# AsherBond/0-kno-vectorx

Measured on AMD Instinct MI355X. Metric: header_range_256 proofs/sec, higher is better.
Workload: dtype u64 (Goldilocks) / u8 (hashes)

## Files before the change

### 0-kno-vectorx_amd/csrc/vx_blake_air.hip

```cpp
#include <string.h>

#include "air_blake.cuh"
#include "vx_internal.h"


static uint8_t compact_mode(uint32_t v) { return v < (1u << 6) ? 0 : v < (1u << 14) ? 1 : v < (1u << 30) ? 2 : 3; }

struct BlockDesc {
    uint64_t msg_off;
    uint32_t t, inc;
    uint32_t D[8];
    uint8_t fin, first, act, mode;
    uint32_t num;
    uint32_t size;
};

__device__ __forceinline__ uint64_t b_rotr(uint64_t x, int n) { return (x >> n) | (x << (64 - n)); }

__device__ __forceinline__ void carries(uint64_t o1, uint64_t o2, uint64_t o3, uint8_t* out) {
    uint64_t lo = (o1 & 0xFFFFFFFFULL) + (o2 & 0xFFFFFFFFULL) + (o3 & 0xFFFFFFFFULL);
    uint64_t klo = lo >> 32;
    uint64_t hi = (o1 >> 32) + (o2 >> 32) + (o3 >> 32) + klo;
    out[0] = (uint8_t)klo;
    out[1] = (uint8_t)(hi >> 32);
}
__device__ __forceinline__ void g_mix(uint64_t* v, int ia, int ib, int ic, int id, uint64_t x, uint64_t y) {
    uint64_t a = v[ia], b = v[ib], c = v[ic], d = v[id];
    uint64_t a1 = a + b + x, d1 = b_rotr(d ^ a1, 32), c1 = c + d1, b1 = b_rotr(b ^ c1, 24);
    uint64_t a2 = a1 + b1 + y, d2 = b_rotr(d1 ^ a2, 16), c2 = c1 + d2, b2 = b_rotr(b1 ^ c2, 63);
    v[ia] = a2, v[ib] = b2, v[ic] = c2, v[id] = d2;
}
__device__ void blake_round(uint64_t* v, const uint64_t* m, int round) {
    const uint8_t* s = blk::ORDER[round + 1];
    for (int k = 0; k < 4; ++k) g_mix(v, k, 4 + k, 8 + k, 12 + k, m[s[2 * k]], m[s[2 * k + 1]]);
    for (int j = 0; j < 4; ++j) g_mix(v, j, 4 + (j + 1) % 4, 8 + (j + 2) % 4, 12 + (j + 3) % 4, m[s[8 + 2 * j]], m[s[8 + 2 * j + 1]]);
}
__device__ void blake_init_v(uint64_t* v, const uint64_t* h, uint64_t t, bool fin) {
    for (int i = 0; i < 8; ++i) v[i] = h[i], v[8 + i] = blk::IV[i];
    v[12] ^= t;
    if (fin) v[14] = ~v[14];
}

__global__ __launch_bounds__(64) void k_blake_chain(const uint8_t* msgs, size_t stride, const uint32_t* sizes, size_t n,
                                                    const uint32_t* block_base, uint64_t* hchain, uint8_t* digests) {
    size_t i = blockIdx.x * (size_t)blockDim.x + threadIdx.x;
    if (i >= n) return;
    const uint64_t* p = (const uint64_t*)(msgs + i * stride);
    const uint32_t len = sizes[i];
    const uint32_t nchunks = len == 0 ? 1 : (len + 127) / 128;
    uint64_t h[8], m[16], v[16];
    for (int k = 0; k < 8; ++k) h[k] = blk::IV[k];
    h[0] ^= 0x01010020ULL;
    for (uint32_t cidx = 0; cidx < nchunks; ++cidx) {
        uint64_t* hc = hchain + 8 * ((size_t)block_base[i] + cidx);
        for (int k = 0; k < 8; ++k) hc[k] = h[k];
        const bool fin = cidx + 1 == nchunks;
        const uint32_t off = 128 * cidx, rem = fin ? len - off : 128;
        for (int k = 0; k < 16; ++k) {
            uint32_t b = 8 * k;
            uint64_t w = 0;
            if (b < rem) {
                w = p[(off >> 3) + k];
                if (rem - b < 8) w &= (1ULL << (8 * (rem - b))) - 1;
            }
            m[k] = w;
        }
        blake_init_v(v, h, fin ? len : off + 128, fin);
        for (int r = 0; r < 12; ++r) blake_round(v, m, r);
        for (int k = 0; k < 8; ++k) h[k] ^= v[k] ^ v[k + 8];
    }
    uint64_t* d = (uint64_t*)(digests + 32 * i);
    d[0] = h[0], d[1] = h[1], d[2] = h[2], d[3] = h[3];
}

#ifndef VX_HIST_COPIES
#define VX_HIST_COPIES 8
#endif
constexpr int HIST_COPIES = VX_HIST_COPIES;
constexpr int SW_CAR = 64, SW_MS = 65, SW_MB = 81, SW_HL = 82, SW_D = 90, SW_FLAGS = 94, SW_TN = 95, SW_WIN = 96, N_STAGE = 97;
struct ExpandEntry {
    uint16_t col;
    uint8_t shift, bits;
};
__global__ __launch_bounds__(256) void k_blake_trace(const uint8_t* msgs, const BlockDesc* descs, const uint64_t* hchain, size_t n_real,
                                                     uint64_t* __restrict__ stage, uint32_t* __restrict__ hist, uint32_t* __restrict__ rc_part, size_t n,
                                                     uint32_t win_off, uint32_t win_len) {
    using namespace blk;
    __shared__ uint32_t rc_lds[256];
    rc_lds[threadIdx.x] = 0;
    __syncthreads();
    const size_t row = blockIdx.x * (size_t)blockDim.x + threadIdx.x;
    const size_t b = row >> 4;
    const int r = (int)(row & 15);
    const BlockDesc d = descs[b];
    uint64_t h[8], m[16], v[16];
    if (b < n_real) {
        for (int k = 0; k < 8; ++k) h[k] = hchain[8 * b + k];
        const uint64_t* p = (const uint64_t*)(msgs + d.msg_off);
        for (int k = 0; k < 16; ++k) {
            uint32_t bb = 8 * k;
            uint64_t w = 0;
            if (bb < d.inc) {
                w = p[k];
                if (d.inc - bb < 8) w &= (1ULL << (8 * (d.inc - bb))) - 1;
            }
            m[k] = w;
        }
    } else {
        for (int k = 0; k < 8; ++k) h[k] = IV[k];
        h[0] ^= 0x01010020ULL;
        for (int k = 0; k < 16; ++k) m[k] = k < 4 ? ((uint64_t)d.D[2 * k] | ((uint64_t)d.D[2 * k + 1] << 32)) : 0;
        m[4] = d.mode == 0 ? 4ULL * d.num : d.mode == 1 ? 4ULL * d.num + 1 : d.mode == 2 ? 4ULL * d.num + 2 : (3ULL | ((uint64_t)d.num << 8));
    }
    auto st = [&](int w) -> uint64_t& { return stage[(size_t)w * n + row]; };
    auto gw = [&](int k, int slot) -> uint64_t& { return st(8 * k + slot); };
    uint32_t* const hc = hist + (size_t)(blockIdx.x % HIST_COPIES) * 131072;
    auto look1 = [&](uint64_t a, uint64_t bq) {
#pragma unroll
        for (int j = 0; j < 8; ++j) atomicAdd(&hc[((a >> (8 * j)) & 0xFF) | (((bq >> (8 * j)) & 0xFF) << 8)], 1u);
    };
    auto look2 = [&](uint64_t a, uint64_t bq) {
#pragma unroll
        for (int j = 0; j < 8; ++j) atomicAdd(&hc[65536 + (((a >> (8 * j)) & 0xFF) | (((bq >> (8 * j)) & 0xFF) << 8))], 1u);
    };
    blake_init_v(v, h, d.t, d.fin);
    uint64_t carw = 0;
    if (r >= 1 && r <= 12) {
        for (int q = 0; q + 1 < r; ++q) blake_round(v, m, q);
        const uint8_t* sg = ORDER[r];
        auto G = [&](int k, uint64_t& va, uint64_t& vb, uint64_t& vc, uint64_t& vd, uint64_t x, uint64_t y) {
            const uint64_t a = va, bq = vb, c = vc, dd = vd;
            const uint64_t a1 = a + bq + x, d1 = b_rotr(dd ^ a1, 32), c1 = c + d1, b1 = b_rotr(bq ^ c1, 24);
            const uint64_t a2 = a1 + b1 + y, d2 = b_rotr(d1 ^ a2, 16), c2 = c1 + d2, b2 = b_rotr(b1 ^ c2, 63);
            gw(k, S_A1) = a1, gw(k, S_D1) = d1, gw(k, S_C1) = c1, gw(k, S_B1) = b1, gw(k, S_A2) = a2, gw(k, S_D2) = d2, gw(k, S_C2) = c2, gw(k, 7) = b1 ^ c2;
            uint8_t car[4];
            carries(a, bq, x, car);
            carries(a1, b1, y, car + 2);
            carw |= ((uint64_t)car[0] | ((uint64_t)car[1] << 2) | ((uint64_t)car[2] << 4) | ((uint64_t)car[3] << 6)) << (8 * k);
            look1(dd, a1), look1(bq, c1), look1(d1, a2), look2(b1, c2);
            va = a2, vb = b2, vc = c2, vd = d2;
        };
        G(0, v[0], v[4], v[8], v[12], m[sg[0]], m[sg[1]]);
        G(1, v[1], v[5], v[9], v[13], m[sg[2]], m[sg[3]]);
        G(2, v[2], v[6], v[10], v[14], m[sg[4]], m[sg[5]]);
        G(3, v[3], v[7], v[11], v[15], m[sg[6]], m[sg[7]]);
        G(4, v[0], v[5], v[10], v[15], m[sg[8]], m[sg[9]]);
        G(5, v[1], v[6], v[11], v[12], m[sg[10]], m[sg[11]]);
        G(6, v[2], v[7], v[8], v[13], m[sg[12]], m[sg[13]]);
        G(7, v[3], v[4], v[9], v[14], m[sg[14]], m[sg[15]]);
    } else {
        for (int w = 0; w < 64; ++w) st(w) = 0;
        if (r == 0) {
            for (int w = 0; w < 16; ++w) {
                const int mm = w & 3;
                if (w < 4) gw(4 + w, S_A2) = v[w];
                else if (w < 8) gw(4 + (mm + 3) % 4, 7) = b_rotr(v[w], 1);
                else if (w < 12) gw(4 + (mm + 2) % 4, S_C2) = v[w];
                else gw(4 + (mm + 1) % 4, S_D2) = v[w];
            }
        } else {
            for (int q = 0; q < 12; ++q) blake_round(v, m, q);
            if (r <= 14)
                for (int w = 0; w < 8; ++w) {
                    const uint64_t u = v[w] ^ v[8 + w];
                    const uint64_t x = r == 13 ? v[w] : u, y = r == 13 ? v[8 + w] : h[w];
                    gw(w, S_D1) = x, gw(w, S_A2) = y, gw(w, S_D2) = b_rotr(x ^ y, 16);
                    look1(x, y);
                }
        }
    }
    st(SW_CAR) = carw;
    uint64_t h_out[8];
    if (r >= 13)
        for (int k = 0; k < 8; ++k) h_out[k] = h[k] ^ v[k] ^ v[k + 8];
    for (int s = 0; s < 16; ++s) st(SW_MS + s) = m[ORDER[r][s]];
    st(SW_MB) = m[r];
#pragma unroll
    for (int j = 0; j < 8; ++j) atomicAdd(&rc_lds[(m[r] >> (8 * j)) & 0xFF], 1u);
    for (int w = 0; w < 8; ++w) st(SW_HL + w) = r <= 13 ? h[w] : (r == 14 ? h_out[w] : (d.fin ? (w == 0 ? IV[0] ^ 0x01010020ULL : IV[w]) : h_out[w]));
    const bool cap = d.act && d.fin;
    for (int j = 0; j < 4; ++j) st(SW_D + j) = (r == 15 && cap) ? h_out[j] : ((uint64_t)d.D[2 * j] | ((uint64_t)d.D[2 * j + 1] << 32));
    uint64_t mk = 0;
    for (int bq = 0; bq < 8; ++bq) mk |= (uint64_t)((uint32_t)(8 * r + bq) < d.inc ? 1 : 0) << bq;
    const uint64_t cnt = d.inc < (uint32_t)(8 * (r + 1)) ? d.inc : (uint32_t)(8 * (r + 1));
    const bool srw = d.first && r >= 4 && r <= 8;
    const uint32_t clen = d.mode == 0 ? 1 : d.mode == 1 ? 2 : d.mode == 2 ? 4 : 5, kof = srw ? 32 + clen : (win_len ? win_off : d.size - 32);
    const uint32_t wlen = (win_len && !srw) ? win_len : 32;
    uint64_t eb = 0;
    for (int bq = 0; bq < 8; ++bq) {
        const uint32_t pos = d.t - d.inc + 8 * r + bq;
        eb |= (uint64_t)((d.act && pos >= kof && pos < kof + wlen && (!win_len || (pos < d.size && !srw))) ? 1 : 0) << bq;
    }
    const uint64_t mdf = d.first ? (uint64_t)(d.mode == 0) | ((uint64_t)(d.mode == 1) << 1) | ((uint64_t)(d.mode == 3) << 2) : 0;
    st(SW_FLAGS) = (uint64_t)d.act | ((uint64_t)d.fin << 1) | ((uint64_t)d.first << 2) | ((uint64_t)(cap ? 1 : 0) << 3) | ((uint64_t)((d.first && d.act) ? 1 : 0) << 4) |
                   (mdf << 5) | ((uint64_t)d.inc << 8) | (cnt << 16) | (mk << 24) | (eb << 32) | ((uint64_t)d.size << 40);
    st(SW_TN) = (uint64_t)d.t | ((uint64_t)d.num << 32);
    st(SW_WIN) = (uint64_t)kof | ((uint64_t)(srw ? 0 : 1) << 32);
    __syncthreads();
    rc_part[(size_t)blockIdx.x * 256 + threadIdx.x] = rc_lds[threadIdx.x];
}
constexpr int EXP_RPL = 8;
__global__ __launch_bounds__(256) void k_blake_expand(const uint64_t* __restrict__ stage, uint64_t* __restrict__ tr, size_t n, const ExpandEntry* __restrict__ ent,
                                                      const uint32_t* __restrict__ off) {
    const int w = blockIdx.y;
    const size_t row0 = (size_t)blockIdx.x * (256 * EXP_RPL) + threadIdx.x;
    uint64_t x[EXP_RPL];
#pragma unroll
    for (int rr = 0; rr < EXP_RPL; ++rr) {
        const size_t row = row0 + 256 * (size_t)rr;
        x[rr] = row < n ? stage[(size_t)w * n + row] : 0;
    }
    for (uint32_t e = off[w]; e < off[w + 1]; ++e) {
        const ExpandEntry E = ent[e];
        const uint64_t mask = E.bits == 64 ? ~0ULL : ((1ULL << E.bits) - 1);
        uint64_t* c = tr + (size_t)E.col * n;
#pragma unroll
        for (int rr = 0; rr < EXP_RPL; ++rr) {
            const size_t row = row0 + 256 * (size_t)rr;
            if (row < n) c[row] = (x[rr] >> E.shift) & mask;
        }
    }
}
static void blake_expand_table(std::vector<ExpandEntry>& ent, std::vector<uint32_t>& off) {
    using namespace blk;
    std::vector<std::vector<ExpandEntry>> per(N_STAGE);
    auto add = [&](int w, int col, int shift, int bits) { per[w].push_back(ExpandEntry{(uint16_t)col, (uint8_t)shift, (uint8_t)bits}); };
    for (int k = 0; k < 8; ++k) {
        for (int slot = 0; slot < 7; ++slot)
            for (int j = 0; j < 8; ++j) add(8 * k + slot, GC(k, slot, j), 8 * j, 8);
        for (int j = 0; j < 8; ++j) add(8 * k + 7, GC(k, S_L, j), 8 * j, 7), add(8 * k + 7, GC(k, S_T, j), 8 * j + 7, 1);
        for (int q = 0; q < 4; ++q) add(SW_CAR, CAR(k, q), 8 * k + 2 * q, 2);
    }
    for (int s = 0; s < 16; ++s) add(SW_MS + s, MS(s, 0), 0, 32), add(SW_MS + s, MS(s, 1), 32, 32);
    for (int j = 0; j < 8; ++j) add(SW_MB, MB0 + j, 8 * j, 8);
    for (int w = 0; w < 8; ++w) add(SW_HL + w, HL(w, 0), 0, 32), add(SW_HL + w, HL(w, 1), 32, 32);
    for (int j = 0; j < 4; ++j) add(SW_D + j, D0 + 2 * j, 0, 32), add(SW_D + j, D0 + 2 * j + 1, 32, 32);
    add(SW_FLAGS, ACT, 0, 1), add(SW_FLAGS, FIN, 1, 1), add(SW_FLAGS, FIRST, 2, 1), add(SW_FLAGS, CAP, 3, 1), add(SW_FLAGS, FA, 4, 1);
    add(SW_FLAGS, INC, 8, 8), add(SW_FLAGS, CNT, 16, 8);
    for (int i = 0; i < 8; ++i) add(SW_FLAGS, IB0 + i, 8 + i, 1), add(SW_FLAGS, MK0 + i, 24 + i, 1), add(SW_FLAGS, E0 + i, 32 + i, 1);
    add(SW_FLAGS, SZ, 40, 24);
    add(SW_FLAGS, MDF0, 5, 1), add(SW_FLAGS, MDF1, 6, 1), add(SW_FLAGS, MDF3, 7, 1);
    add(SW_WIN, KOF, 0, 24), add(SW_WIN, TR, 32, 1);
    add(SW_TN, T, 0, 32), add(SW_TN, NUM, 32, 32);
    for (int i = 0; i < 32; ++i) add(SW_TN, TB0 + i, i, 1);
    off.assign(1, 0);
    for (auto& v : per) {
        ent.insert(ent.end(), v.begin(), v.end());
        off.push_back((uint32_t)ent.size());
    }
}
__global__ __launch_bounds__(256) void k_blake_mult(const uint32_t* hist, const uint32_t* rc_part, uint64_t* tr, size_t n) {
    const size_t row = blockIdx.x * (size_t)blockDim.x + threadIdx.x;
    if (row >= n) return;
    uint64_t m1 = 0, m2 = 0;
    if (row < 65536)
        for (int cpy = 0; cpy < HIST_COPIES; ++cpy) m1 += hist[(size_t)cpy * 131072 + row], m2 += hist[(size_t)cpy * 131072 + 65536 + row];
    if (row < 256)
        for (size_t b = 0; b < n / 256; ++b) m1 += rc_part[b * 256 + row];
    tr[(size_t)blk::M1 * n + row] = m1;
    tr[(size_t)blk::M2 * n + row] = m2;
}

struct AuxArgs {
    const uint64_t* tr;
    uint64_t* aux;
    uint64_t* part;
    size_t n;
    gl2 beta, gamma;
    uint64_t first_number, tree_size, bus_on;
};
#ifndef VX_AUX_WAVES
#define VX_AUX_WAVES 4
#endif
__global__ __launch_bounds__(256) __attribute__((amdgpu_waves_per_eu(VX_AUX_WAVES, VX_AUX_WAVES))) void k_blake_aux(AuxArgs a) {
    using namespace blk;
    const size_t n = a.n, i = blockIdx.x * (size_t)blockDim.x + threadIdx.x;
    const int unit = blockIdx.y;
    if (i >= n) return;
    const size_t ip = (i + n - 1) & (n - 1);
    const int rl = (int)(ip & 15);
    const bool g_on = rl <= 11, m3 = rl <= 13;
    const bus::Bus<gl2> bus(a.beta.a, a.beta.b, a.gamma.a, a.gamma.b);
    auto N = [&](int col) -> uint64_t { return a.tr[(size_t)col * n + i]; };
    auto L = [&](int col) -> uint64_t { return a.tr[(size_t)col * n + ip]; };
    auto store = [&](int e, gl2 h) {
        a.aux[(size_t)(2 * e) * n + i] = h.a;
        a.aux[(size_t)(2 * e + 1) * n + i] = h.b;
    };
    gl2 hsum{0, 0};
    auto four = [&](gl2* p, gl2* s, int e0) {
        const gl2 c1 = gl2_mul(p[0], p[1]), c2 = gl2_mul(c1, p[2]), c3 = gl2_mul(c2, p[3]);
        gl2 inv = gl2_inv(c3);
        const gl2 i3 = gl2_mul(inv, c2);
        inv = gl2_mul(inv, p[3]);
        const gl2 i2 = gl2_mul(inv, c1);
        inv = gl2_mul(inv, p[2]);
        const gl2 i1 = gl2_mul(inv, p[0]), i0 = gl2_mul(inv, p[1]);
        const gl2 iq[4] = {i0, i1, i2, i3};
#pragma unroll
        for (int q = 0; q < 4; ++q) {
            const gl2 h = gl2_mul(s[q], iq[q]);
            store(e0 + q, h);
            hsum = gl2_add(hsum, h);
        }
    };
    if (unit < 8) {
        const int k = unit;
        const gl2 bt2 = bus.t2_base();
        auto out_byte_loc = [&](int w, int j) -> uint64_t {
            const int m = w & 3;
            if (w < 8) {
// ... 105 lines not shown
__global__ __launch_bounds__(256) void k_blake_aux_z(const uint64_t* part, uint64_t* aux, size_t n) {
    using namespace blk;
    const size_t i = blockIdx.x * (size_t)blockDim.x + threadIdx.x;
    if (i >= n) return;
    const size_t ip = (i + n - 1) & (n - 1);
    uint64_t sa = 0, sb = 0;
#pragma unroll
    for (int u = 0; u < 9; ++u) sa = gl_add(sa, part[(size_t)(2 * u) * n + i]), sb = gl_add(sb, part[(size_t)(2 * u + 1) * n + i]);
    aux[(size_t)(2 * ZZ) * n + ip] = gl_sub(sa, aux[(size_t)(2 * HT) * n + ip]);
    aux[(size_t)(2 * ZZ + 1) * n + ip] = gl_sub(sb, aux[(size_t)(2 * HT + 1) * n + ip]);
}

int32_t BlakeAir::gen_aux(vx_ctx* ctx, const uint64_t* trace, int log_n, const uint64_t* chal, const uint64_t* pub, uint64_t* aux, uint64_t* aux_pub) {
    const size_t n = (size_t)1 << log_n;
    uint64_t* part = (uint64_t*)vx_pool_alloc(ctx, 18 * n * 8);
    if (!part) return vx_fail(ctx, VX_ERR_OOM, "blake aux: out of device memory");
    AuxArgs a{trace, aux, part, n, gl2{chal[0], chal[1]}, gl2{chal[2], chal[3]}, pub[19] == 1 ? pub[18] : pub[16], pub[18], pub[19]};
    hipLaunchKernelGGL(k_blake_aux, dim3((unsigned)((n + 255) / 256), 9), dim3(256), 0, ctx->stream, a);
    hipLaunchKernelGGL(k_blake_aux_z, dim3((unsigned)((n + 255) / 256)), dim3(256), 0, ctx->stream, (const uint64_t*)part, aux, n);
    const hipError_t e = hipGetLastError();
    vx_pool_free(ctx, part);
    if (e != hipSuccess) return vx_fail(ctx, VX_ERR_DEVICE, "blake aux: %s", hipGetErrorString(e));
    return vx_bus_close_dev(ctx, aux + (size_t)(2 * blk::ZZ) * n, log_n, aux_pub);
}

extern "C" {

int32_t vx_blake_chain_trace(vx_ctx* ctx, const vx_buf* headers, size_t stride, const uint32_t* sizes, size_t n_headers,
                             const uint8_t trusted_hash[32], uint32_t first_block_number, uint32_t tree_size, uint32_t window_offset, uint32_t window_length,
                             int log_n, vx_buf* trace_out, uint64_t public_inputs_out[20], uint8_t* digests_out) {
    if (!ctx || !headers || !sizes || !trusted_hash || !trace_out || !public_inputs_out) return VX_ERR_ARG;
    VX_CHECK(stride % 128 == 0 && stride > 0, "blake trace: stride %zu must be a positive multiple of 128", stride);
    VX_CHECK(n_headers >= 1 && n_headers * stride <= headers->n * 8, "blake trace: headers exceed the buffer");
    VX_CHECK(log_n >= blk::TABLE_LOG && log_n <= 24, "blake trace: log_n %d out of range [16, 24] (the trace holds one copy of the 2^16-row lookup tables)", log_n);
    VX_CHECK((uint64_t)first_block_number + n_headers <= (1ULL << 32), "blake trace: block numbers %u.. overflow 32 bits", first_block_number);
    VX_CHECK(!window_length || (n_headers == 1 && !tree_size && window_offset >= 72 && (uint64_t)window_offset + window_length < (1u << 24)),
             "blake trace: a byte window (offset %u, length %u) goes with one header, no Merkle tree, and starts behind the state root", window_offset, window_length);
    VX_CHECK(window_length || window_offset == 0 || (tree_size && window_offset < first_block_number), "blake trace: a leaf offset (%u) goes with tree_size != 0", window_offset);
    const size_t n = (size_t)1 << log_n, n_blocks = n >> 4;
    VX_CHECK(trace_out->n >= n * blk::COLS, "blake trace: trace buffer holds %zu < %zu elements", trace_out->n, n * (size_t)blk::COLS);
    std::vector<uint32_t> base(n_headers);
    size_t n_real = 0;
    for (size_t i = 0; i < n_headers; ++i) {
        const uint32_t clen = (uint32_t[]){1, 2, 4, 5}[compact_mode(first_block_number + (uint32_t)i)];
        VX_CHECK(sizes[i] <= stride && sizes[i] >= 32 + clen && sizes[i] < (1u << 24), "blake trace: header %zu has size %u", i, sizes[i]);
        VX_CHECK(!tree_size || sizes[i] >= 104,
                 "blake trace: header %zu has size %u (shorter than 104 bytes its state root and data root would share trace rows; no Avail header is)", i, sizes[i]);
        base[i] = (uint32_t)n_real;
        n_real += (sizes[i] + 127) / 128;
    }
    VX_CHECK(n_real <= n_blocks, "blake trace: %zu compressions do not fit 2^%d rows (%zu blocks)", n_real, log_n, n_blocks);
    const size_t w_sizes = (n_headers * 4 + 7) / 8, w_dig = n_headers * 4, w_hc = n_real * 8;
    const size_t w_desc = (n_blocks * sizeof(BlockDesc) + 7) / 8;
    const size_t w_hist = (size_t)HIST_COPIES * 65536 + n / 2;
    std::vector<ExpandEntry> ent;
    std::vector<uint32_t> eoff;
    blake_expand_table(ent, eoff);
    VX_CHECK(ent.size() == (size_t)blk::COLS - 2, "blake trace: expansion table covers %zu of %d columns", ent.size(), blk::COLS - 2);
    const size_t w_ent = (ent.size() * sizeof(ExpandEntry) + 7) / 8, w_eoff = (eoff.size() * 4 + 7) / 8, w_stage = (size_t)N_STAGE * n;
    uint64_t* sc;
    VX_TRY(vx_scratch(ctx, 2 * w_sizes + w_dig + w_hc + w_desc + w_hist + w_ent + w_eoff + w_stage, &sc));
    uint32_t* d_sizes = (uint32_t*)sc;
    uint32_t* d_base = (uint32_t*)(sc + w_sizes);
    uint8_t* d_dig = (uint8_t*)(sc + 2 * w_sizes);
    uint64_t* d_hc = sc + 2 * w_sizes + w_dig;
    BlockDesc* d_desc = (BlockDesc*)(d_hc + w_hc);
    uint32_t* d_hist = (uint32_t*)(d_hc + w_hc + w_desc);
    ExpandEntry* d_ent = (ExpandEntry*)(d_hc + w_hc + w_desc + w_hist);
    uint32_t* d_eoff = (uint32_t*)(d_hc + w_hc + w_desc + w_hist + w_ent);
    uint64_t* d_stage = d_hc + w_hc + w_desc + w_hist + w_ent + w_eoff;
    VX_HIP(hipMemcpyAsync(d_ent, ent.data(), ent.size() * sizeof(ExpandEntry), hipMemcpyHostToDevice, ctx->stream));
    VX_HIP(hipMemcpyAsync(d_eoff, eoff.data(), eoff.size() * 4, hipMemcpyHostToDevice, ctx->stream));
    VX_HIP(hipMemcpyAsync(d_sizes, sizes, n_headers * 4, hipMemcpyHostToDevice, ctx->stream));
    VX_HIP(hipMemcpyAsync(d_base, base.data(), n_headers * 4, hipMemcpyHostToDevice, ctx->stream));
    hipLaunchKernelGGL(k_blake_chain, dim3((unsigned)((n_headers + 63) / 64)), dim3(64), 0, ctx->stream, (const uint8_t*)headers->d,
                       stride, (const uint32_t*)d_sizes, n_headers, (const uint32_t*)d_base, d_hc, d_dig);
    VX_HIP(hipGetLastError());
    std::vector<uint8_t> dig(32 * n_headers);
    VX_HIP(hipMemcpyAsync(dig.data(), d_dig, dig.size(), hipMemcpyDeviceToHost, ctx->stream));
    VX_HIP(hipStreamSynchronize(ctx->stream));
    std::vector<BlockDesc> descs(n_blocks);
    uint8_t D[32];
    memcpy(D, trusted_hash, 32);
    size_t bi = 0;
    for (size_t i = 0; i < n_headers; ++i) {
        const uint32_t nch = (sizes[i] + 127) / 128;
        for (uint32_t cidx = 0; cidx < nch; ++cidx, ++bi) {
            BlockDesc& d = descs[bi];
            memset(&d, 0, sizeof d);
            d.fin = cidx + 1 == nch;
            d.first = cidx == 0;
            d.act = 1;
            d.inc = d.fin ? sizes[i] - 128 * cidx : 128;
            d.t = d.fin ? sizes[i] : 128 * (cidx + 1);
            d.msg_off = i * stride + 128 * (size_t)cidx;
            d.num = first_block_number + (uint32_t)i;
            d.mode = compact_mode(d.num);
            d.size = sizes[i];
            memcpy(d.D, D, 32);
        }
        memcpy(D, dig.data() + 32 * i, 32);
    }
    for (; bi < n_blocks; ++bi) {
        BlockDesc& d = descs[bi];
        memset(&d, 0, sizeof d);
        d.fin = d.first = 1;
        d.act = 0;
        d.inc = d.t = d.size = 40;
        d.msg_off = ~0ULL;
        d.num = first_block_number + (uint32_t)n_headers - 1;
        d.mode = compact_mode(d.num);
        memcpy(d.D, D, 32);
    }
    VX_HIP(hipMemcpyAsync(d_desc, descs.data(), n_blocks * sizeof(BlockDesc), hipMemcpyHostToDevice, ctx->stream));
    VX_HIP(hipMemsetAsync(d_hist, 0, (size_t)HIST_COPIES * 65536 * 8, ctx->stream));
    hipLaunchKernelGGL(k_blake_trace, dim3((unsigned)((n + 255) / 256)), dim3(256), 0, ctx->stream, (const uint8_t*)headers->d,
                       (const BlockDesc*)d_desc, (const uint64_t*)d_hc, n_real, d_stage, d_hist, d_hist + (size_t)HIST_COPIES * 131072, n, window_offset, window_length);
    VX_HIP(hipGetLastError());
    hipLaunchKernelGGL(k_blake_expand, dim3((unsigned)((n + 256 * EXP_RPL - 1) / (256 * EXP_RPL)), N_STAGE), dim3(256), 0, ctx->stream,
                       (const uint64_t*)d_stage, trace_out->d, n, (const ExpandEntry*)d_ent, (const uint32_t*)d_eoff);
    VX_HIP(hipGetLastError());
    hipLaunchKernelGGL(k_blake_mult, dim3((unsigned)((n + 255) / 256)), dim3(256), 0, ctx->stream, (const uint32_t*)d_hist, (const uint32_t*)(d_hist + (size_t)HIST_COPIES * 131072), trace_out->d, n);
    VX_HIP(hipGetLastError());
    VX_HIP(hipStreamSynchronize(ctx->stream));
    for (int j = 0; j < 8; ++j) {
        uint32_t a, b;
        memcpy(&a, trusted_hash + 4 * j, 4);
        memcpy(&b, D + 4 * j, 4);
        public_inputs_out[j] = a;
        public_inputs_out[8 + j] = b;
    }
    public_inputs_out[16] = first_block_number;
    public_inputs_out[17] = first_block_number + (uint64_t)n_headers - 1;
    public_inputs_out[18] = window_length ? window_offset : (tree_size ? (uint64_t)first_block_number - window_offset : 0);
    public_inputs_out[19] = window_length ? 2 : (tree_size ? 1 : 0);
    if (digests_out) memcpy(digests_out, dig.data(), dig.size());
    return VX_OK;
}

}
```

### 0-kno-vectorx_amd/csrc/vx_ed_air.hip

```cpp
#include <string.h>

#include "air_ed.cuh"
#include "ed25519.cuh"
#include "vx_internal.h"

namespace {
using namespace edc;

struct EdSlot {
    int32_t xa[16], ya[16], x3[16], y3[16], xr[16], yr[16];
    int32_t wxa[16], wya[16], wxr[16], wyr[16];
    int32_t hl[32], qq[17], hr[16], hw[16], crlo[32], crhi[32];
    uint8_t cxa[16], cya[16], cxr[16], cyr[16], chr[16];
    uint8_t dig[64];
    uint32_t s[8], h[8];
    uint32_t sign_a, sign_r, sg, cnt, aidx, pad;
};

__device__ void limbs16(const ed::U256& x, int32_t* out) {
    for (int i = 0; i < 8; ++i) out[2 * i] = x.w[i] & 0xFFFF, out[2 * i + 1] = x.w[i] >> 16;
}
__device__ void canon_witness(const int32_t* x, int t, int32_t* w, uint8_t* cy) {
    int32_t borrow = 0;
    for (int k = 0; k < 16; ++k) {
// ... 200 lines not shown
        if (k == 0) row[C(1, 0)] = in.qq[16], row[C(12, 0)] = 1, row[C(13, 0)] = 1;
        for (int j = k; j < 64; j += 16) row[BYA(j)] = in.dig[j], row[BYB(j)] = 256 * (int32_t)in.dig[j];
    }
    registers(0, 0, 0);
    int32_t X = 0, Y = one_k, Z = one_k, lah = 0;
    for (int r = 2; r < 255; ++r) {
        row += COLS;
        const int bit = 252 - (r - 2);
        const int32_t bs = (in.s[bit >> 5] >> (bit & 31)) & 1, bh = (in.h[bit >> 5] >> (bit & 31)) & 1;
        lah = ((bit == 252 || (bit & 15) == 15) ? 0 : 2 * lah) + bh;
        registers(bs, bh, lah);
        const int32_t w11 = bs & bh, w10 = bs - w11, w01 = bh - w11, w00 = 1 - bs - bh + w11;
        const int32_t s0 = w00 * one_k + w10 * kk(K_BC0) + w01 * (ya + xa) + w11 * (y3 - x3), s1 = w00 * one_k + w10 * kk(K_BC1) + w01 * (ya - xa) + w11 * (y3 + x3);
        const int32_t s2 = w10 * kk(K_BC2) + w01 * nt + w11 * bt;
        const int32_t q = pick(X, Y, Z, X + Y);
        (void)finish(gi, fold(q, q), true, 0);
        const int32_t c0 = Cs[0][k], c1 = Cs[1][k], c2 = Cs[2][k], c3 = Cs[3][k];
        const int32_t E = c3 - c0 - c1, G = c1 - c0, F = G - 2 * c2, H = -c0 - c1;
        (void)finish(4 + gi, fold(pick(E, G, E, F), pick(F, H, H, G)), true, 0);
        const int32_t c4 = Cs[0][k], c5 = Cs[1][k], c6 = Cs[2][k], c7 = Cs[3][k];
        (void)finish(gi < 3 ? 8 + gi : -1, fold(pick(c5 - c4, c5 + c4, c6, 0), pick(s0, s1, s2, 0)), true, 0);
        const int32_t c8 = Cs[0][k], c9 = Cs[1][k], c10 = Cs[2][k];
        const int32_t E2 = c9 - c8, F2 = 2 * c7 - c10, G2 = 2 * c7 + c10, H2 = c9 + c8;
        (void)finish(gi < 3 ? 11 + gi : -1, fold(pick(E2, G2, F2, 0), pick(F2, H2, G2, 0)), true, 0);
        X = Cs[0][k], Y = Cs[1][k], Z = Cs[2][k];
    }
    row += COLS;
    clear();
    {
        const int32_t xr = in.xr[k], yr = in.yr[k];
        const int64_t f = fold(pick(xr, yr, 0, 0), pick(Z, Z, 0, 0));
        (void)finish(gi < 2 ? gi : -1, f - pick(X, Y, 0, 0), false, pick(xr, yr, 0, 0));
        if (gi == 0) {
            row[C(2, k)] = in.wxr[k], row[C(3, k)] = in.wyr[k];
            if (k < 15) row[RL(2, k)] = in.cxr[k], row[RL(3, k)] = in.cyr[k];
            if (k == 0) row[RH(2, 0)] = xr >> 1;
        }
        registers((int32_t)in.sign_r, 0, lah);
    }
}

__global__ __launch_bounds__(256) void k_ed_expand(const int32_t* stage, uint64_t* trace, size_t n, size_t k_active) {
    __shared__ int32_t tile[64][65];
    const size_t row0 = blockIdx.x * (size_t)64, slot = row0 >> 8, src0 = (slot < k_active ? slot : k_active) * 256 + (row0 & 255);
    const int col0 = blockIdx.y * 64, tx = threadIdx.x & 63, ty = threadIdx.x >> 6;
    for (int r = ty; r < 64; r += 4) tile[r][tx] = col0 + tx < COLS ? stage[(src0 + r) * COLS + col0 + tx] : 0;
    __syncthreads();
    for (int c = ty; c < 64; c += 4) {
        if (col0 + c >= COLS) break;
        const int32_t v = tile[tx][c];
        trace[(size_t)(col0 + c) * n + row0 + tx] = v < 0 ? GL_P - (uint64_t)(-(int64_t)v) : (uint64_t)v;
    }
}
constexpr int ED_HIST_COPIES = 32;
__global__ __launch_bounds__(256) void k_ed_hist(const int32_t* stage, size_t k_active, uint32_t idle_weight, uint32_t* hist) {
    const size_t row = blockIdx.x;
    const uint32_t w = (row >> 8) < k_active ? 1u : idle_weight;
    uint32_t* h = hist + (size_t)(blockIdx.x % ED_HIST_COPIES) * 65536;
    for (int col = threadIdx.x; col < CELLS; col += 256) atomicAdd(&h[(uint32_t)stage[row * COLS + col] & 65535u], w);
}
__global__ __launch_bounds__(256) void k_ed_mult(const uint32_t* hist, uint64_t* mult_col) {
    const size_t i = blockIdx.x * (size_t)blockDim.x + threadIdx.x;
    uint64_t s = 0;
    for (int c = 0; c < ED_HIST_COPIES; ++c) s += hist[(size_t)c * 65536 + i];
    mult_col[i] = s;
}

__global__ __launch_bounds__(256) void k_ed_inv_table(gl2 beta, gl2 gamma, gl2* inv) {
    const uint32_t v = blockIdx.x * blockDim.x + threadIdx.x;
    const bus::Bus<gl2> bus(beta.a, beta.b, gamma.a, gamma.b);
    inv[v] = gl2_inv(bus.r16(bus.r16_base(), v));
}
struct EdAuxArgs {
    const uint64_t* tr;
    uint64_t* aux;
    const gl2* inv;
    size_t n;
    gl2 beta, gamma;
    uint64_t bus_on;
};
__global__ __launch_bounds__(256) void k_ed_aux(EdAuxArgs a) {
    const size_t i = blockIdx.x * (size_t)blockDim.x + threadIdx.x, n = a.n;
    if (i >= n) return;
    auto T = [&](int col) -> uint64_t { return a.tr[(size_t)col * n + i]; };
    gl2 hsum{0, 0};
#pragma unroll 4
    for (int e = 0; e < N_RANGE; ++e) {
        const gl2 h = gl2_add(a.inv[T(2 * e) & 65535], a.inv[T(2 * e + 1) & 65535]);
        a.aux[(size_t)(2 * e) * n + i] = h.a, a.aux[(size_t)(2 * e + 1) * n + i] = h.b;
        hsum = gl2_add(hsum, h);
    }
    const int r = (int)(i & 255);
    gl2 hb[N_BUS];
    for (int b = 0; b < N_BUS; ++b) hb[b] = gl2{0, 0};
    if ((r == 0 || r == 1 || r == 255) && a.bus_on && T(SG)) {
        const bus::Bus<gl2> bus(a.beta.a, a.beta.b, a.gamma.a, a.gamma.b);
        const uint64_t slot4 = 4 * (uint64_t)(i >> 8), sign = T(BS), aidx4 = 4 * T(AIDX);
        auto enc = [&](int g, int k) -> uint64_t { return k < 15 ? T(C(g, k)) : T(C(g, 15)) + 32768 * sign; };
        auto neg = [](gl2 x) -> gl2 { return gl2{gl_neg(x.a), gl_neg(x.b)}; };
        if (r == 0) {
            for (int b = 0; b < 4; ++b)
                hb[b] = neg(gl2_inv(bus.key(aidx4 + b, enc(7, 4 * b) | (enc(7, 4 * b + 1) << 16), enc(7, 4 * b + 2) | (enc(7, 4 * b + 3) << 16))));
            for (int b = 0; b < 2; ++b)
                hb[4 + b] = gl2_inv(bus.ed_msg(slot4 + b + 2, enc(7, 8 * b) | (enc(7, 8 * b + 1) << 16) | (enc(7, 8 * b + 2) << 32),
                                       enc(7, 8 * b + 3) | (enc(7, 8 * b + 4) << 16) | (enc(7, 8 * b + 5) << 32), enc(7, 8 * b + 6) | (enc(7, 8 * b + 7) << 16)));
        } else if (r == 1) {
            auto dh = [&](int q) -> uint64_t {
                if (q >= 16) return 0;
                const int b0 = 8 * (q >> 1) + ((q & 1) ? 0 : 4);
                return (T(BYA(b0)) << 24) | (T(BYA(b0 + 1)) << 16) | (T(BYA(b0 + 2)) << 8) | T(BYA(b0 + 3));
            };
            for (int b = 0; b < 6; ++b) hb[b] = neg(gl2_inv(bus.ed_digest(2 * slot4 + b, dh(3 * b), dh(3 * b + 1), dh(3 * b + 2))));
        } else {
            for (int b = 0; b < 2; ++b)
                hb[4 + b] = gl2_inv(bus.ed_msg(slot4 + b, enc(1, 8 * b) | (enc(1, 8 * b + 1) << 16) | (enc(1, 8 * b + 2) << 32),
                                       enc(1, 8 * b + 3) | (enc(1, 8 * b + 4) << 16) | (enc(1, 8 * b + 5) << 32), enc(1, 8 * b + 6) | (enc(1, 8 * b + 7) << 16)));
        }
    }
    for (int b = 0; b < N_BUS; ++b) {
        a.aux[(size_t)(2 * (HB0 + b)) * n + i] = hb[b].a, a.aux[(size_t)(2 * (HB0 + b) + 1) * n + i] = hb[b].b;
        hsum = gl2_add(hsum, hb[b]);
    }
    const gl2 ht = gl2_scale(a.inv[i & 65535], T(MULT));
    a.aux[(size_t)(2 * HT) * n + i] = ht.a, a.aux[(size_t)(2 * HT + 1) * n + i] = ht.b;
    const gl2 inc = gl2_sub(hsum, ht);
    a.aux[(size_t)(2 * ZZ) * n + i] = inc.a, a.aux[(size_t)(2 * ZZ + 1) * n + i] = inc.b;
}
}

int32_t vx_ed_air_gen_aux(vx_ctx* ctx, const uint64_t* trace, int log_n, const uint64_t* chal, const uint64_t* pub, uint64_t* aux, uint64_t* aux_pub) {
    const size_t n = (size_t)1 << log_n;
    gl2* inv = (gl2*)vx_pool_alloc(ctx, 65536 * sizeof(gl2));
    if (!inv) return vx_fail(ctx, VX_ERR_OOM, "ed aux: out of device memory");
    EdAuxArgs a{trace, aux, inv, n, gl2{chal[0], chal[1]}, gl2{chal[2], chal[3]}, pub[1]};
    hipLaunchKernelGGL(k_ed_inv_table, dim3(256), dim3(256), 0, ctx->stream, a.beta, a.gamma, inv);
    hipLaunchKernelGGL(k_ed_aux, dim3((unsigned)((n + 255) / 256)), dim3(256), 0, ctx->stream, a);
    const hipError_t e = hipGetLastError();
    vx_pool_free(ctx, inv);
    if (e != hipSuccess) return vx_fail(ctx, VX_ERR_DEVICE, "ed aux: %s", hipGetErrorString(e));
    return vx_bus_close_dev(ctx, aux + (size_t)(2 * ZZ) * n, log_n, aux_pub);
}

int32_t vx_ed_trace_dev(vx_ctx* ctx, const uint8_t* pubkeys, const uint8_t* sigs, const uint8_t* msg, uint32_t msg_len, const uint8_t* signed_flags, size_t n_sigs,
                        int log_n, uint64_t bus_on, uint64_t* trace_d, uint64_t pub_out[2]) {
    const size_t n = (size_t)1 << log_n, m = n >> 8;
    VX_CHECK(log_n >= 16 && log_n <= 20, "ed trace: log_n %d out of range [16, 20] (the trace holds one copy of the 2^16-row range table)", log_n);
    VX_CHECK(msg_len <= 64, "ed trace: message of %u bytes (the precommit has 53)", msg_len);
    std::vector<uint32_t> idx;
    for (size_t s = 0; s < n_sigs; ++s)
        if (signed_flags[s]) idx.push_back((uint32_t)s);
    const size_t k = idx.size(), k4 = k + 1;
    VX_CHECK(k < m, "ed trace: %zu signatures do not fit the %zu slots of 2^%d rows (one slot stays idle)", k, m - 1, log_n);
    const size_t w_keys = 4 * n_sigs + 1, w_sigs = 8 * n_sigs + 1, w_msg = 8, w_idx = (k + 1) / 2 + 1, w_slots = ((k + 1) * sizeof(EdSlot) + 7) / 8;
    const size_t w_hist = (size_t)ED_HIST_COPIES * 65536 / 2;
    uint64_t* sc;
    VX_TRY(vx_scratch(ctx, w_keys + w_sigs + w_msg + w_idx + 1 + w_slots + w_hist, &sc));
    uint8_t* d_keys = (uint8_t*)sc;
    uint8_t* d_sigs = (uint8_t*)(sc + w_keys);
    uint8_t* d_msg = (uint8_t*)(sc + w_keys + w_sigs);
    uint32_t* d_idx = (uint32_t*)(sc + w_keys + w_sigs + w_msg);
    uint32_t* d_bad = (uint32_t*)(sc + w_keys + w_sigs + w_msg + w_idx);
    EdSlot* d_slots = (EdSlot*)(sc + w_keys + w_sigs + w_msg + w_idx + 1);
    uint32_t* d_hist = (uint32_t*)(sc + w_keys + w_sigs + w_msg + w_idx + 1 + w_slots);
    if (n_sigs) {
        VX_HIP(hipMemcpyAsync(d_keys, pubkeys, 32 * n_sigs, hipMemcpyHostToDevice, ctx->stream));
        VX_HIP(hipMemcpyAsync(d_sigs, sigs, 64 * n_sigs, hipMemcpyHostToDevice, ctx->stream));
    }
    if (k) VX_HIP(hipMemcpyAsync(d_idx, idx.data(), k * 4, hipMemcpyHostToDevice, ctx->stream));
    VX_HIP(hipMemcpyAsync(d_msg, msg, msg_len, hipMemcpyHostToDevice, ctx->stream));
    VX_HIP(hipMemsetAsync(d_bad, 0, 8, ctx->stream));
    VX_HIP(hipMemsetAsync(d_hist, 0, w_hist * 8, ctx->stream));
    int32_t* stage = (int32_t*)vx_pool_alloc(ctx, k4 * 256 * (size_t)COLS * 4);
    if (!stage) return vx_fail(ctx, VX_ERR_OOM, "ed trace: out of device memory");
    hipLaunchKernelGGL(k_ed_slots, dim3((unsigned)((k + 1 + 63) / 64)), dim3(64), 0, ctx->stream, d_keys, d_sigs, d_msg, msg_len, (const uint32_t*)d_idx, k, d_slots, d_bad);
    hipLaunchKernelGGL(k_ed_rows, dim3((unsigned)k4), dim3(64), 0, ctx->stream, (const EdSlot*)d_slots, stage, k, d_bad);
    hipLaunchKernelGGL(k_ed_expand, dim3((unsigned)(n / 64), (COLS + 63) / 64), dim3(256), 0, ctx->stream, (const int32_t*)stage, trace_d, n, k);
    hipLaunchKernelGGL(k_ed_hist, dim3((unsigned)((k + 1) * 256)), dim3(256), 0, ctx->stream, (const int32_t*)stage, k, (uint32_t)(m - k), d_hist);
    hipLaunchKernelGGL(k_ed_mult, dim3(256), dim3(256), 0, ctx->stream, (const uint32_t*)d_hist, trace_d + (size_t)MULT * n);
    const hipError_t e = hipGetLastError();
    vx_pool_free(ctx, stage);
    if (e != hipSuccess) return vx_fail(ctx, VX_ERR_DEVICE, "ed trace: %s", hipGetErrorString(e));
    uint32_t bad = 0;
    VX_HIP(hipMemcpyAsync(&bad, d_bad, 4, hipMemcpyDeviceToHost, ctx->stream));
    VX_HIP(hipStreamSynchronize(ctx->stream));
    if (bad) return vx_fail(ctx, VX_ERR_STATEMENT, "ed trace: a signed slot does not verify (undecodable key / R, or [S]B != R + [h]A)");
    pub_out[0] = k, pub_out[1] = bus_on;
    return VX_OK;
}

extern "C" int32_t vx_ed_trace(vx_ctx* ctx, const uint8_t* pubkeys, const uint8_t* signatures, const uint8_t* message, uint32_t message_len, const uint8_t* signed_flags,
                               size_t n_signatures, int log_n, uint32_t bus_on, vx_buf* trace_out, uint64_t public_inputs_out[2]) {
    if (!ctx || !message || !trace_out || !public_inputs_out || (n_signatures && (!pubkeys || !signatures || !signed_flags))) return VX_ERR_ARG;
    VX_CHECK(log_n >= 16 && log_n <= 20 && trace_out->n >= ((size_t)COLS << log_n), "ed trace: trace buffer holds %zu elements, 2^%d rows need %zu", trace_out->n, log_n,
             (size_t)COLS << log_n);
    return vx_ed_trace_dev(ctx, pubkeys, signatures, message, message_len, signed_flags, n_signatures, log_n, bus_on ? 1 : 0, trace_out->d, public_inputs_out);
}
```

Baseline: 8.396.

## Replace global atomic lookup histograms with partitioned LDS histogram kernels

Moves the blake lookup-multiplicity counting out of the trace kernel into a separate count kernel. That kernel rereads the stage buffer and accumulates each 2^15-key partition of the histogram in shared memory, then writes per-slice partials that the mult kernel sums. The ed histogram gets the same partitioned LDS scheme, plus per-thread merging of duplicate keys before the atomics. The aim is to remove heavily contended global atomics and the histogram memsets. The cost is extra passes that reread the stage, since each partition workgroup scans every row.

```diff
diff --git a/0-kno-vectorx_amd/csrc/vx_blake_air.hip b/0-kno-vectorx_amd/csrc/vx_blake_air.hip
--- a/0-kno-vectorx_amd/csrc/vx_blake_air.hip
+++ b/0-kno-vectorx_amd/csrc/vx_blake_air.hip
@@ -73,22 +73,14 @@
     d[0] = h[0], d[1] = h[1], d[2] = h[2], d[3] = h[3];
 }
 
-#ifndef VX_HIST_COPIES
-#define VX_HIST_COPIES 8
-#endif
-constexpr int HIST_COPIES = VX_HIST_COPIES;
 constexpr int SW_CAR = 64, SW_MS = 65, SW_MB = 81, SW_HL = 82, SW_D = 90, SW_FLAGS = 94, SW_TN = 95, SW_WIN = 96, N_STAGE = 97;
 struct ExpandEntry {
     uint16_t col;
     uint8_t shift, bits;
 };
 __global__ __launch_bounds__(256) void k_blake_trace(const uint8_t* msgs, const BlockDesc* descs, const uint64_t* hchain, size_t n_real,
-                                                     uint64_t* __restrict__ stage, uint32_t* __restrict__ hist, uint32_t* __restrict__ rc_part, size_t n,
-                                                     uint32_t win_off, uint32_t win_len) {
+                                                     uint64_t* __restrict__ stage, size_t n, uint32_t win_off, uint32_t win_len) {
     using namespace blk;
-    __shared__ uint32_t rc_lds[256];
-    rc_lds[threadIdx.x] = 0;
-    __syncthreads();
     const size_t row = blockIdx.x * (size_t)blockDim.x + threadIdx.x;
     const size_t b = row >> 4;
     const int r = (int)(row & 15);
@@ -114,15 +106,6 @@
     }
     auto st = [&](int w) -> uint64_t& { return stage[(size_t)w * n + row]; };
     auto gw = [&](int k, int slot) -> uint64_t& { return st(8 * k + slot); };
-    uint32_t* const hc = hist + (size_t)(blockIdx.x % HIST_COPIES) * 131072;
-    auto look1 = [&](uint64_t a, uint64_t bq) {
-#pragma unroll
-        for (int j = 0; j < 8; ++j) atomicAdd(&hc[((a >> (8 * j)) & 0xFF) | (((bq >> (8 * j)) & 0xFF) << 8)], 1u);
-    };
-    auto look2 = [&](uint64_t a, uint64_t bq) {
-#pragma unroll
-        for (int j = 0; j < 8; ++j) atomicAdd(&hc[65536 + (((a >> (8 * j)) & 0xFF) | (((bq >> (8 * j)) & 0xFF) << 8))], 1u);
-    };
     blake_init_v(v, h, d.t, d.fin);
     uint64_t carw = 0;
     if (r >= 1 && r <= 12) {
@@ -137,7 +120,6 @@
             carries(a, bq, x, car);
             carries(a1, b1, y, car + 2);
             carw |= ((uint64_t)car[0] | ((uint64_t)car[1] << 2) | ((uint64_t)car[2] << 4) | ((uint64_t)car[3] << 6)) << (8 * k);
-            look1(dd, a1), look1(bq, c1), look1(d1, a2), look2(b1, c2);
             va = a2, vb = b2, vc = c2, vd = d2;
         };
         G(0, v[0], v[4], v[8], v[12], m[sg[0]], m[sg[1]]);
@@ -165,7 +147,6 @@
                     const uint64_t u = v[w] ^ v[8 + w];
                     const uint64_t x = r == 13 ? v[w] : u, y = r == 13 ? v[8 + w] : h[w];
                     gw(w, S_D1) = x, gw(w, S_A2) = y, gw(w, S_D2) = b_rotr(x ^ y, 16);
-                    look1(x, y);
                 }
         }
     }
@@ -175,8 +156,6 @@
         for (int k = 0; k < 8; ++k) h_out[k] = h[k] ^ v[k] ^ v[k + 8];
     for (int s = 0; s < 16; ++s) st(SW_MS + s) = m[ORDER[r][s]];
     st(SW_MB) = m[r];
-#pragma unroll
-    for (int j = 0; j < 8; ++j) atomicAdd(&rc_lds[(m[r] >> (8 * j)) & 0xFF], 1u);
     for (int w = 0; w < 8; ++w) st(SW_HL + w) = r <= 13 ? h[w] : (r == 14 ? h_out[w] : (d.fin ? (w == 0 ? IV[0] ^ 0x01010020ULL : IV[w]) : h_out[w]));
     const bool cap = d.act && d.fin;
     for (int j = 0; j < 4; ++j) st(SW_D + j) = (r == 15 && cap) ? h_out[j] : ((uint64_t)d.D[2 * j] | ((uint64_t)d.D[2 * j + 1] << 32));
@@ -196,8 +175,6 @@
                    (mdf << 5) | ((uint64_t)d.inc << 8) | (cnt << 16) | (mk << 24) | (eb << 32) | ((uint64_t)d.size << 40);
     st(SW_TN) = (uint64_t)d.t | ((uint64_t)d.num << 32);
     st(SW_WIN) = (uint64_t)kof | ((uint64_t)(srw ? 0 : 1) << 32);
-    __syncthreads();
-    rc_part[(size_t)blockIdx.x * 256 + threadIdx.x] = rc_lds[threadIdx.x];
 }
 constexpr int EXP_RPL = 8;
 __global__ __launch_bounds__(256) void k_blake_expand(const uint64_t* __restrict__ stage, uint64_t* __restrict__ tr, size_t n, const ExpandEntry* __restrict__ ent,
@@ -249,14 +226,67 @@
         off.push_back((uint32_t)ent.size());
     }
 }
-__global__ __launch_bounds__(256) void k_blake_mult(const uint32_t* hist, const uint32_t* rc_part, uint64_t* tr, size_t n) {
+#ifndef VX_PART_BITS
+#define VX_PART_BITS 15
+#endif
+constexpr int PART_BITS = VX_PART_BITS, PART = 1 << PART_BITS, PARTS = 65536 >> PART_BITS;
+constexpr int CNT_WGS = 256, CNT_THREADS = 1024;
+constexpr int CNT_SLICES1 = 3 * CNT_WGS / (4 * PARTS), CNT_SLICES2 = CNT_WGS / (4 * PARTS);
+static_assert(PART_BITS >= 12 && PART_BITS <= 15 && CNT_SLICES2 >= 1, "a part is 16 .. 128 KiB of LDS");
+__global__ __launch_bounds__(CNT_THREADS) void k_blake_count(const uint64_t* __restrict__ stage, size_t n, uint32_t* __restrict__ partial) {
+    using namespace blk;
+    __shared__ uint32_t h[PART];
+    const bool t2 = blockIdx.x >= PARTS * CNT_SLICES1;
+    const uint32_t wg = t2 ? blockIdx.x - PARTS * CNT_SLICES1 : blockIdx.x, slices = t2 ? CNT_SLICES2 : CNT_SLICES1;
+    const uint32_t sub = wg / slices, slice = wg % slices;
+    for (int i = threadIdx.x; i < PART; i += CNT_THREADS) h[i] = 0;
+    __syncthreads();
+    auto look = [&](uint64_t a, uint64_t b) {
+#pragma unroll
+        for (int j = 0; j < 8; ++j) {
+            const uint32_t key = (uint32_t)((a >> (8 * j)) & 0xFF) | ((uint32_t)((b >> (8 * j)) & 0xFF) << 8);
+            if ((key >> PART_BITS) == sub) atomicAdd(&h[key & (PART - 1)], 1u);
+        }
+    };
+    auto rotl = [](uint64_t x, int s) -> uint64_t { return (x << s) | (x >> (64 - s)); };
+    for (size_t row = (size_t)slice * CNT_THREADS + threadIdx.x; row < n; row += (size_t)slices * CNT_THREADS) {
+        const int r = (int)(row & 15);
+        auto st = [&](int w) -> uint64_t { return stage[(size_t)w * n + row]; };
+        const bool g_row = r >= 1 && r <= 12;
+        if (t2) {
+            if (g_row) {
+#pragma unroll
+                for (int k = 0; k < 8; ++k) look(st(8 * k + S_B1), st(8 * k + S_C2));
+            }
+        } else {
+            if (g_row) {
+#pragma unroll 4
+                for (int k = 0; k < 8; ++k) {
+                    const uint64_t a1 = st(8 * k + S_A1), d1 = st(8 * k + S_D1), c1 = st(8 * k + S_C1), b1 = st(8 * k + S_B1), a2 = st(8 * k + S_A2);
+                    look(rotl(d1, 32) ^ a1, a1), look(rotl(b1, 24) ^ c1, c1), look(d1, a2);
+                }
+            } else if (r == 13 || r == 14) {
+#pragma unroll
+                for (int w = 0; w < 8; ++w) look(st(8 * w + S_D1), st(8 * w + S_A2));
+            }
+            if (sub == 0) look(st(SW_MB), 0);
+        }
+    }
+    __syncthreads();
+    uint32_t* out = partial + (t2 ? (size_t)65536 * CNT_SLICES1 : 0) + ((size_t)sub * slices + slice) * PART;
+    for (int i = threadIdx.x; i < PART; i += CNT_THREADS) out[i] = h[i];
+}
+__global__ __launch_bounds__(256) void k_blake_mult(const uint32_t* __restrict__ partial, uint64_t* tr, size_t n) {
     const size_t row = blockIdx.x * (size_t)blockDim.x + threadIdx.x;
     if (row >= n) return;
     uint64_t m1 = 0, m2 = 0;
-    if (row < 65536)
-        for (int cpy = 0; cpy < HIST_COPIES; ++cpy) m1 += hist[(size_t)cpy * 131072 + row], m2 += hist[(size_t)cpy * 131072 + 65536 + row];
-    if (row < 256)
-        for (size_t b = 0; b < n / 256; ++b) m1 += rc_part[b * 256 + row];
+    if (row < 65536) {
+        const size_t sub = row >> PART_BITS, bin = row & (PART - 1);
+        const uint32_t* p1 = partial + sub * CNT_SLICES1 * PART + bin;
+        const uint32_t* p2 = partial + (size_t)65536 * CNT_SLICES1 + sub * CNT_SLICES2 * PART + bin;
+        for (int s = 0; s < CNT_SLICES1; ++s) m1 += p1[(size_t)s * PART];
+        for (int s = 0; s < CNT_SLICES2; ++s) m2 += p2[(size_t)s * PART];
+    }
     tr[(size_t)blk::M1 * n + row] = m1;
     tr[(size_t)blk::M2 * n + row] = m2;
 }
@@ -468,7 +498,7 @@
     VX_CHECK(n_real <= n_blocks, "blake trace: %zu compressions do not fit 2^%d rows (%zu blocks)", n_real, log_n, n_blocks);
     const size_t w_sizes = (n_headers * 4 + 7) / 8, w_dig = n_headers * 4, w_hc = n_real * 8;
     const size_t w_desc = (n_blocks * sizeof(BlockDesc) + 7) / 8;
-    const size_t w_hist = (size_t)HIST_COPIES * 65536 + n / 2;
+    const size_t w_hist = (size_t)65536 * (CNT_SLICES1 + CNT_SLICES2) / 2;
     std::vector<ExpandEntry> ent;
     std::vector<uint32_t> eoff;
     blake_expand_table(ent, eoff);
@@ -529,14 +559,15 @@
         memcpy(d.D, D, 32);
     }
     VX_HIP(hipMemcpyAsync(d_desc, descs.data(), n_blocks * sizeof(BlockDesc), hipMemcpyHostToDevice, ctx->stream));
-    VX_HIP(hipMemsetAsync(d_hist, 0, (size_t)HIST_COPIES * 65536 * 8, ctx->stream));
     hipLaunchKernelGGL(k_blake_trace, dim3((unsigned)((n + 255) / 256)), dim3(256), 0, ctx->stream, (const uint8_t*)headers->d,
-                       (const BlockDesc*)d_desc, (const uint64_t*)d_hc, n_real, d_stage, d_hist, d_hist + (size_t)HIST_COPIES * 131072, n, window_offset, window_length);
+                       (const BlockDesc*)d_desc, (const uint64_t*)d_hc, n_real, d_stage, n, window_offset, window_length);
+    VX_HIP(hipGetLastError());
+    hipLaunchKernelGGL(k_blake_count, dim3(PARTS * (CNT_SLICES1 + CNT_SLICES2)), dim3(CNT_THREADS), 0, ctx->stream, (const uint64_t*)d_stage, n, d_hist);
     VX_HIP(hipGetLastError());
     hipLaunchKernelGGL(k_blake_expand, dim3((unsigned)((n + 256 * EXP_RPL - 1) / (256 * EXP_RPL)), N_STAGE), dim3(256), 0, ctx->stream,
                        (const uint64_t*)d_stage, trace_out->d, n, (const ExpandEntry*)d_ent, (const uint32_t*)d_eoff);
     VX_HIP(hipGetLastError());
-    hipLaunchKernelGGL(k_blake_mult, dim3((unsigned)((n + 255) / 256)), dim3(256), 0, ctx->stream, (const uint32_t*)d_hist, (const uint32_t*)(d_hist + (size_t)HIST_COPIES * 131072), trace_out->d, n);
+    hipLaunchKernelGGL(k_blake_mult, dim3((unsigned)((n + 255) / 256)), dim3(256), 0, ctx->stream, (const uint32_t*)d_hist, trace_out->d, n);
     VX_HIP(hipGetLastError());
     VX_HIP(hipStreamSynchronize(ctx->stream));
     for (int j = 0; j < 8; ++j) {
diff --git a/0-kno-vectorx_amd/csrc/vx_ed_air.hip b/0-kno-vectorx_amd/csrc/vx_ed_air.hip
--- a/0-kno-vectorx_amd/csrc/vx_ed_air.hip
+++ b/0-kno-vectorx_amd/csrc/vx_ed_air.hip
@@ -276,17 +276,43 @@
         trace[(size_t)(col0 + c) * n + row0 + tx] = v < 0 ? GL_P - (uint64_t)(-(int64_t)v) : (uint64_t)v;
     }
 }
-constexpr int ED_HIST_COPIES = 32;
-__global__ __launch_bounds__(256) void k_ed_hist(const int32_t* stage, size_t k_active, uint32_t idle_weight, uint32_t* hist) {
-    const size_t row = blockIdx.x;
-    const uint32_t w = (row >> 8) < k_active ? 1u : idle_weight;
-    uint32_t* h = hist + (size_t)(blockIdx.x % ED_HIST_COPIES) * 65536;
-    for (int col = threadIdx.x; col < CELLS; col += 256) atomicAdd(&h[(uint32_t)stage[row * COLS + col] & 65535u], w);
-}
-__global__ __launch_bounds__(256) void k_ed_mult(const uint32_t* hist, uint64_t* mult_col) {
+#ifndef VX_ED_PART_BITS
+#define VX_ED_PART_BITS 14
+#endif
+constexpr int ED_PART_BITS = VX_ED_PART_BITS, ED_PART = 1 << ED_PART_BITS, ED_PARTS = 65536 >> ED_PART_BITS;
+constexpr int ED_HIST_WGS = 128, ED_SLICES = ED_HIST_WGS / ED_PARTS, ED_HIST_THREADS = 1024, ED_HIST_UNROLL = 8;
+static_assert(ED_PART_BITS >= 12 && ED_PART_BITS <= 15, "a part is 16 .. 128 KiB of LDS");
+__global__ __launch_bounds__(ED_HIST_THREADS) void k_ed_hist(const int32_t* __restrict__ stage, size_t k_active, uint32_t idle_weight, uint32_t* __restrict__ partial) {
+    __shared__ uint32_t h[ED_PART];
+    const uint32_t sub = blockIdx.x / ED_SLICES, slice = blockIdx.x % ED_SLICES;
+    for (int i = threadIdx.x; i < ED_PART; i += ED_HIST_THREADS) h[i] = 0;
+    __syncthreads();
+    const uint32_t items = (uint32_t)((k_active + 1) * (256 / ED_HIST_UNROLL) * CELLS);
+    for (uint32_t item = slice * ED_HIST_THREADS + threadIdx.x; item < items; item += ED_SLICES * ED_HIST_THREADS) {
+        const uint32_t chunk = item / CELLS, col = item - chunk * CELLS;
+        const int32_t* p = stage + (size_t)chunk * ED_HIST_UNROLL * COLS + col;
+        const uint32_t w = chunk / (256 / ED_HIST_UNROLL) < k_active ? 1u : idle_weight;
+        uint32_t v[ED_HIST_UNROLL], c[ED_HIST_UNROLL];
+#pragma unroll
+        for (int u = 0; u < ED_HIST_UNROLL; ++u) v[u] = (uint32_t)p[(size_t)u * COLS] & 65535u, c[u] = w;
+#pragma unroll
+        for (int u = 1; u < ED_HIST_UNROLL; ++u)
+#pragma unroll
+            for (int t = 0; t < u; ++t)
+                if (c[t] && v[t] == v[u]) c[t] += c[u], c[u] = 0;
+#pragma unroll
+        for (int u = 0; u < ED_HIST_UNROLL; ++u)
+            if (c[u] && (v[u] >> ED_PART_BITS) == sub) atomicAdd(&h[v[u] & (ED_PART - 1)], c[u]);
+    }
+    __syncthreads();
+    uint32_t* out = partial + ((size_t)sub * ED_SLICES + slice) * ED_PART;
+    for (int i = threadIdx.x; i < ED_PART; i += ED_HIST_THREADS) out[i] = h[i];
+}
+__global__ __launch_bounds__(256) void k_ed_mult(const uint32_t* __restrict__ partial, uint64_t* mult_col) {
     const size_t i = blockIdx.x * (size_t)blockDim.x + threadIdx.x;
+    const uint32_t* p = partial + (i >> ED_PART_BITS) * ED_SLICES * ED_PART + (i & (ED_PART - 1));
     uint64_t s = 0;
-    for (int c = 0; c < ED_HIST_COPIES; ++c) s += hist[(size_t)c * 65536 + i];
+    for (int c = 0; c < ED_SLICES; ++c) s += p[(size_t)c * ED_PART];
     mult_col[i] = s;
 }
 
@@ -376,7 +402,7 @@
     const size_t k = idx.size(), k4 = k + 1;
     VX_CHECK(k < m, "ed trace: %zu signatures do not fit the %zu slots of 2^%d rows (one slot stays idle)", k, m - 1, log_n);
     const size_t w_keys = 4 * n_sigs + 1, w_sigs = 8 * n_sigs + 1, w_msg = 8, w_idx = (k + 1) / 2 + 1, w_slots = ((k + 1) * sizeof(EdSlot) + 7) / 8;
-    const size_t w_hist = (size_t)ED_HIST_COPIES * 65536 / 2;
+    const size_t w_hist = (size_t)ED_SLICES * 65536 / 2;
     uint64_t* sc;
     VX_TRY(vx_scratch(ctx, w_keys + w_sigs + w_msg + w_idx + 1 + w_slots + w_hist, &sc));
     uint8_t* d_keys = (uint8_t*)sc;
@@ -393,13 +419,12 @@
     if (k) VX_HIP(hipMemcpyAsync(d_idx, idx.data(), k * 4, hipMemcpyHostToDevice, ctx->stream));
     VX_HIP(hipMemcpyAsync(d_msg, msg, msg_len, hipMemcpyHostToDevice, ctx->stream));
     VX_HIP(hipMemsetAsync(d_bad, 0, 8, ctx->stream));
-    VX_HIP(hipMemsetAsync(d_hist, 0, w_hist * 8, ctx->stream));
     int32_t* stage = (int32_t*)vx_pool_alloc(ctx, k4 * 256 * (size_t)COLS * 4);
     if (!stage) return vx_fail(ctx, VX_ERR_OOM, "ed trace: out of device memory");
     hipLaunchKernelGGL(k_ed_slots, dim3((unsigned)((k + 1 + 63) / 64)), dim3(64), 0, ctx->stream, d_keys, d_sigs, d_msg, msg_len, (const uint32_t*)d_idx, k, d_slots, d_bad);
     hipLaunchKernelGGL(k_ed_rows, dim3((unsigned)k4), dim3(64), 0, ctx->stream, (const EdSlot*)d_slots, stage, k, d_bad);
     hipLaunchKernelGGL(k_ed_expand, dim3((unsigned)(n / 64), (COLS + 63) / 64), dim3(256), 0, ctx->stream, (const int32_t*)stage, trace_d, n, k);
-    hipLaunchKernelGGL(k_ed_hist, dim3((unsigned)((k + 1) * 256)), dim3(256), 0, ctx->stream, (const int32_t*)stage, k, (uint32_t)(m - k), d_hist);
+    hipLaunchKernelGGL(k_ed_hist, dim3(ED_HIST_WGS), dim3(ED_HIST_THREADS), 0, ctx->stream, (const int32_t*)stage, k, (uint32_t)(m - k), d_hist);
     hipLaunchKernelGGL(k_ed_mult, dim3(256), dim3(256), 0, ctx->stream, (const uint32_t*)d_hist, trace_d + (size_t)MULT * n);
     const hipError_t e = hipGetLastError();
     vx_pool_free(ctx, stage);
```

After: 8.616, median of 6. 2.6% higher.
